# mfkiwl/coxgraph

Hardware: AMD Instinct MI355X
Metric: 640x480 depth frames/sec fused (TSDF, 5 cm voxels) per node; submap registrations/sec reported alongside (higher is better)
Workload: dtype f32; 1 GPU; configs[1]: 1 client per GPU, 640x480 synthetic depth stream, 5 cm voxels, merged integrator semantics (the reference's configured method is fast; bit-exact vs CPU oracle), points resident in HBM; points_per_frame=307200, method=merged, clients=1

## Files before the change

coxgraph_amd/csrc/cox_integrator.hip:

```cpp
#include <hip/hip_runtime.h>

#include <algorithm>
#include <chrono>
#include <cmath>
#include <cstring>
#include <limits>
#include <new>
#include <string>
#include <vector>

#include "../../include/coxgraph_hip_history.h"
#include "../../include/coxgraph_hip_selftest.h"
#include "cox_host.hpp"
#include "cox_plan.hpp"
#include "cox_sort.hpp"
#include "cox_threads.hpp"

using namespace cox;
using cox_plan::IntegratorPlan;
using cox_plan::LayerUpdate;

#include "cox_frame.hpp"
#include "cox_raygen.hpp"
#include "cox_walk.hpp"
#include "cox_pieces.hpp"
#include "cox_fast.hpp"
#include "cox_apply_records.hpp"
#include "cox_apply_tile.hpp"
#include "cox_frontend.hpp"

static_assert(cox_plan::kAxisCapSmall == kAxisCapSmall && cox_plan::kTileShift == kTileShift && cox_plan::kBigChunk == kBigChunk &&
                  cox_plan::kBigChunkMin == kBigChunkMin && cox_plan::kFastMaxRounds == kFastMaxRounds && cox_plan::kFastShortMax == kFastShortMax &&
                  cox_plan::kFastRelaxGroups == kFastRelaxGroups && cox_plan::kCopyGroups == kCopyGroups,
              "cox_plan.hpp decides with the kernels' own constants");

constexpr int kStatRing = 8;
constexpr int kFrameSets = 6;
constexpr int kStageSets = 3;
constexpr int kInputSets = kFrameSets;
using cox_plan::kNumStages;

struct FrameSet {
  FrameParams* d_params = nullptr;
  Counters* cnt = nullptr;
  RayArrays rays{};
  u64* fh_keys = nullptr;
  u32* fh_first = nullptr;
  hipEvent_t done = nullptr;
  hipEvent_t params_copied = nullptr;
  hipEvent_t hand[kNumStages - 1] = {};
  bool used = false;
};
struct BundleSet {
  u32 *pslot = nullptr, *skey[2] = {nullptr, nullptr}, *sval[2] = {nullptr, nullptr}, *bstart = nullptr;
  u32 *hrank = nullptr, *head = nullptr;
  SortInfo* sort_info = nullptr;
  hipEvent_t done = nullptr;
  bool used = false;
};
struct RecordSet {
  u32 *rec_key[2] = {nullptr, nullptr}, *rec_ray[2] = {nullptr, nullptr};
  u32 *piece_front = nullptr, *piece_back = nullptr, *piece_wsum = nullptr;
  uint8_t* lin8 = nullptr;
  u32 *pkey[2] = {nullptr, nullptr}, *pstart[2] = {nullptr, nullptr}, *prl[2] = {nullptr, nullptr};
  u64* pbkey = nullptr;
  u32 *plen = nullptr, *pdest = nullptr;
  u32* touched_slots = nullptr;
// ... 158 lines not shown
  if (I->submitter) {
    I->submitter->wait_outstanding(0);
    const int st = I->submitter->take_status();
    if (st != COX_OK) return st;
  }
  for (int k = 0; k < kNumStages; ++k)
    if (I->st[k] && (k == 0 || I->st[k] != I->st[k - 1])) COX_HIP(hipStreamSynchronize(I->st[k]));
  if (I->st_alt) COX_HIP(hipStreamSynchronize(I->st_alt));
  if (I->st_in) COX_HIP(hipStreamSynchronize(I->st_in));
  if (I->obs) COX_TRY(cox_internal_obs_wait(I->obs));
  return COX_OK;
}

static void drop_graphs(cox_integrator* I) {
  for (auto& row : I->graphs)
    for (hipGraphExec_t& g : row) {
      if (g) (void)hipGraphExecDestroy(g);
      g = nullptr;
    }
}

static int alloc_ray_sets(cox_integrator* I, u32 cap) {
  for (FrameSet& F : I->fs) {
    RayArrays& R = F.rays;
    for (float** p : {&R.px, &R.py, &R.pz, &R.w}) COX_TRY(dev_realloc(I, p, cap));
    for (u32** p : {&R.color, &R.flags, &R.nsteps, &R.rec_off, &R.pbound, &R.piece_off}) COX_TRY(dev_realloc(I, p, cap));
    COX_TRY(dev_realloc(I, &R.key, cap));
    COX_TRY(dev_realloc(I, &R.q, static_cast<size_t>(cap) * 8));
    COX_TRY(dev_realloc(I, &F.fh_keys, static_cast<size_t>(I->fh_cap) + I->fh_cap / 2 + 1));
    F.fh_first = reinterpret_cast<u32*>(F.fh_keys + I->fh_cap);
    COX_HIP(hipMemset(F.fh_keys, 0xFF, sizeof(u64) * I->fh_cap + sizeof(u32) * I->fh_cap));
  }
  for (BundleSet& B : I->bs) {
    for (u32** p : {&B.pslot, &B.skey[0], &B.sval[0], &B.skey[1], &B.sval[1], &B.hrank, &B.bstart}) COX_TRY(dev_realloc(I, p, cap));
    COX_TRY(dev_realloc(I, &B.head, static_cast<size_t>(4) * (cap / kHeadTile + 1)));
  }
  for (int k = 0; k < kInputSets; ++k) {
    COX_TRY(dev_realloc(I, &I->own_xyz[k], static_cast<size_t>(cap) * 3));
    COX_TRY(dev_realloc(I, &I->own_rgba[k], static_cast<size_t>(cap) * 4));
    COX_TRY(dev_realloc(I, &I->own_depth[k], cap));
    COX_TRY(dev_realloc(I, &I->own_depth_rgba[k], static_cast<size_t>(cap) * 4));
  }
  COX_TRY(dev_realloc(I, &I->depth_flag, cap));
  COX_TRY(alloc_sort_ws(I, &I->sort_pts, cap));
  COX_TRY(alloc_sort_ws(I, &I->sort_pts_alt, cap));
  for (ScanWorkspace* ws : {&I->scanws_a, &I->scanws_b, &I->scanws_f}) COX_TRY(dev_realloc(I, &ws->block_sums, scan_num_blocks(cap) + 2));
  return COX_OK;
}
static int alloc_record_sets(cox_integrator* I) {
  const bool pieces = I->plan.walks_pieces(), expand = I->plan.expands_pieces();
  const u32 rcap = I->rcap, piece_cap = I->piece_cap, wave_cap = rcap / 64 + 2;
  for (RecordSet& S : I->rs) {
    if (pieces) {
      COX_TRY(dev_realloc(I, &S.lin8, static_cast<size_t>(piece_cap) * 32));
      for (u32** p : {&S.pkey[0], &S.pstart[0], &S.prl[0], &S.pkey[1], &S.pstart[1], &S.prl[1]}) COX_TRY(dev_realloc(I, p, piece_cap));
    }
    if (expand) {
      COX_TRY(dev_realloc(I, &S.pbkey, piece_cap));
      COX_TRY(dev_realloc(I, &S.plen, piece_cap));
      COX_TRY(dev_realloc(I, &S.pdest, piece_cap));
      S.big_chunk_cap = static_cast<u32>(rcap / kBigChunkMin) + kBigCap + 1u;
      COX_TRY(dev_realloc(I, &S.big_chunks, S.big_chunk_cap));
    }
    if (!pieces || expand) {
      COX_TRY(dev_realloc(I, &S.rec_key[0], rcap));
      COX_TRY(dev_realloc(I, &S.rec_ray[0], rcap));
    }
// ... 142 lines not shown
        return e;
      }
      hipEvent_t e = nullptr;
      return hipEventCreate(&e) == hipSuccess ? e : nullptr;
    };
    e0 = take();
    e1 = take();
    if (!e0 || !e1) {
      e0 = e1 = nullptr;
      return;
    }
    (void)hipEventRecord(e0, s);
  }
  ~TimedRegion() {
    if (!e0) return;
    (void)hipEventRecord(e1, s);
    I->class_events[cls].emplace_back(e0, e1);
  }
};

struct StageCtx {
  cox_integrator* I;
  FrameSet* F;
  BundleSet* B;
  RecordSet* S;
  int slot;
  u64 frame;
  const u32* n_dev = nullptr;
};

static LayerView layer_view(const cox_layer* Lh) {
  return LayerView{Lh->voxels, Lh->ht_keys, Lh->ht_vals, Lh->ht_stamp, Lh->ht_ord, Lh->block_keys, Lh->d_nblocks, Lh->ht_cap - 1, static_cast<u32>(Lh->capacity)};
}
static int points_sort_passes(const cox_integrator* I) { return (ceil_log2(next_pow2(static_cast<u64>(I->pcap) + 1)) + 1 + 10) / 11; }

static int stage_hash(const StageCtx& c, hipStream_t s) {
  cox_integrator* I = c.I;
  FrameSet& F = *c.F;
  BundleSet& B = *c.B;
  const bool by_value = (I->method == COX_METHOD_MERGED) && !I->graphs_on;
  if (!by_value) {
    COX_HIP(hipMemcpyAsync(F.d_params, &I->h_params[c.slot], sizeof(FrameParams), hipMemcpyHostToDevice, s));
    if (c.n_dev) hipLaunchKernelGGL(k_params_count, dim3(1), dim3(1), 0, s, F.d_params, c.n_dev);
  }
  COX_HIP(hipMemsetAsync(F.cnt, 0, sizeof(Counters), s));
  if (I->method == COX_METHOD_MERGED) {
    const u32 n = I->pcap;
    {
      TimedRegion t(I, COX_KC_BUNDLE_HASH, s);
      const bool self_clean = !I->cfg.enable_anti_grazing;
      if (!self_clean) COX_HIP(hipMemsetAsync(F.fh_keys, 0xFF, sizeof(u64) * I->fh_cap + sizeof(u32) * I->fh_cap, s));
      hipLaunchKernelGGL(k_bundle_insert, grid_for(n), dim3(256), 0, s, F.d_params, I->h_params[c.slot], by_value ? 1 : 0, c.n_dev, F.fh_keys, F.fh_first,
                         I->fh_cap - 1, B.pslot, F.cnt);
    }
  }
  return COX_OK;
}
static int stage_point_sort(const StageCtx& c, hipStream_t s) {
  cox_integrator* I = c.I;
  FrameSet& F = *c.F;
  BundleSet& B = *c.B;
  if (I->method == COX_METHOD_MERGED) {
    const u32 n = I->pcap;
    const SortWorkspace& ws = (I->st_alt && (c.slot & 1)) ? I->sort_pts_alt : I->sort_pts;
    const bool counted = static_cast<u64>(n) <= static_cast<u64>(kRsMaxTiles) * kRsTile;
    {
      TimedRegion t(I, COX_KC_BUNDLE_HASH, s);
      hipLaunchKernelGGL(k_bundle_keys, grid_for(n, kHeadTile), dim3(kKeysThreads), 0, s, F.d_params, F.fh_keys, F.fh_first, B.pslot, B.skey[0], B.sval[0], B.hrank, B.head,
                         B.sort_info, counted ? ws.counts : nullptr, ws.totals);
    }
    const bool self_clean = !I->cfg.enable_anti_grazing;
    const BundleBounds bounds{F.d_params, B.head, B.hrank, B.pslot, B.bstart, F.cnt, self_clean ? F.fh_keys : nullptr, F.fh_first, I->fh_cap - 1};
    TimedRegion t(I, COX_KC_POINT_SORT, s);
    (void)radix_sort_pairs<11, BundleBounds>(B.skey[0], B.sval[0], B.skey[1], B.sval[1], &F.d_params->n_points, n, n, 0, true, points_sort_passes(I), ws, B.sort_info,
                                             s, nullptr, nullptr, counted, bounds);
  }
  return COX_OK;
}
static FrameBlocks frame_blocks(const cox_integrator* I, const RecordSet& S) { return FrameBlocks{S.ft_keys, S.ft_ord, S.touched_slots, I->layer->ht_cap - 1}; }
static void record_walk(const StageCtx& c, hipStream_t s) {
  cox_integrator* I = c.I;
  const IntegratorPlan& P = I->plan;
  FrameSet& F = *c.F;
  RecordSet& S = *c.S;
  const u32 fh_mask = I->fh_cap - 1;
  const FrameBlocks FB = frame_blocks(I, S);
  if (P.small_axis_cap)
    hipLaunchKernelGGL(k_touch_wave<kAxisCapSmall>, dim3(P.grid_touch), dim3(256), 0, s, F.d_params, F.rays, FB, S.rec_key[1], I->rcap, F.cnt, F.fh_keys, fh_mask);
  else
    hipLaunchKernelGGL(k_touch_wave<kAxisCapLarge>, dim3(2048), dim3(256), 0, s, F.d_params, F.rays, FB, S.rec_key[1], I->rcap, F.cnt, F.fh_keys, fh_mask);
  hipLaunchKernelGGL(k_emit_wave, dim3(P.grid_touch), dim3(256), 0, s, F.d_params, F.rays, FB, S.rec_key[1], S.rec_key[0], S.rec_ray[0], I->rcap, F.cnt, S.sort_info,
                     F.fh_keys, fh_mask, P.emit_flags());
}
static bool binds_in_apply(const cox_integrator* I) { return I->method == COX_METHOD_MERGED && I->plan.layer_update == LayerUpdate::RecordTiles; }
static void bind_blocks(const StageCtx& c, hipStream_t s) {
  cox_integrator* I = c.I;
  if (binds_in_apply(I)) return;
  hipLaunchKernelGGL(k_bind_blocks, dim3(16), dim3(256), 0, s, layer_view(I->layer), frame_blocks(I, *c.S), c.S->ord_info, c.F->cnt, I->layer->d_err);
}
static int stage_merge(const StageCtx& c, hipStream_t s) {
  cox_integrator* I = c.I;
  FrameSet& F = *c.F;
  BundleSet& B = *c.B;
  const u32 n = I->pcap;
  if (I->method == COX_METHOD_MERGED) {
    BundleView V{{B.skey[0], B.skey[1]}, {B.sval[0], B.sval[1]}, B.sort_info};
    {
      TimedRegion t(I, COX_KC_MERGE, s);
      hipLaunchKernelGGL(k_bundle_merge, dim3(I->plan.grid_merge), dim3(256), 0, s, F.d_params, V, B.bstart, F.rays, F.cnt,
                         I->plan.walks_pieces() ? (I->plan.small_axis_cap ? kAxisCapSmall : kAxisCapLarge) : 0u);
    }
    const bool odd = I->st_alt && (c.slot & 1);
    const ScanWorkspace& ws = odd ? I->scanws_a : I->scanws_b;
    if (!I->plan.walks_pieces()) {
      hipLaunchKernelGGL(k_scan_small, dim3(1), dim3(1024), 0, s, F.rays.nsteps, F.rays.rec_off, &F.cnt->n_ray_slots, I->pcap, &F.cnt->n_records);
    } else if (I->plan.small_axis_cap) {
      hipLaunchKernelGGL(k_scan_small2, dim3(1), dim3(1024), 0, s, F.rays.nsteps, F.rays.rec_off, &F.cnt->n_records, F.rays.pbound, F.rays.piece_off,
                         &F.cnt->n_piece_slots, &F.cnt->n_ray_slots, I->pcap);
    } else {
      exclusive_scan_u32(F.rays.nsteps, F.rays.rec_off, &F.cnt->n_ray_slots, I->pcap, I->pcap, &F.cnt->n_records, ws, s);
      exclusive_scan_u32(F.rays.pbound, F.rays.piece_off, &F.cnt->n_ray_slots, I->pcap, I->pcap, &F.cnt->n_piece_slots, ws, s);
    }
  } else {
    hipLaunchKernelGGL(k_rays_simple, grid_for(n), dim3(256), 0, s, F.d_params, F.rays, F.cnt);
  }
  return COX_OK;
}
static int stage_touch(const StageCtx& c, hipStream_t s) {
  cox_integrator* I = c.I;
  const IntegratorPlan& P = I->plan;
  FrameSet& F = *c.F;
  RecordSet& S = *c.S;
  const LayerView L = layer_view(I->layer);
  const u32 fh_mask = I->fh_cap - 1;
  if (P.walk_on_raygen) {
    bind_blocks(c, s);
    return COX_OK;
  }
  TimedRegion t_walk(I, COX_KC_TOUCH_EMIT, s);
  if (P.walks_pieces()) {
    const PieceArrays PA{S.pkey[0], S.pstart[0], S.prl[0], S.pbkey};
#define COX_LAUNCH_WALK(CAP, DEFER)                                                                                                                       \
  hipLaunchKernelGGL((k_touch_pieces<CAP, DEFER>), dim3(2048), dim3(256), 0, s, F.d_params, F.rays, L, S.touched_slots, S.lin8, PA, I->rcap, I->piece_cap, \
// ... 1179 lines not shown
```

coxgraph_amd/csrc/cox_plan.hpp:

```cpp
#pragma once
#include <algorithm>
#include <cmath>
#include <cstdint>
#include <cstdio>
#include <cstdlib>
#include <cstring>
#include <string>

#include "../../include/coxgraph_hip.h"

namespace cox_plan {

#define COX_PLAN_SWITCHES(X)                                                                                                                   \
  X(APPLY) X(APPLY_WAVE) X(BIG_CHUNK) X(BUCKETS) X(COPY_THREADS) X(DEBUG) X(DEPTH_CONVERT) X(FAST_CAP) X(FAST_FENCE) X(FAST_GROUPS)             \
  X(FAST_ROUNDS) X(FAST_SEQUENTIAL) X(FAST_STREAMS) X(GRAPH) X(GRID_APPLY) X(GRID_APPLY_WAVE) X(GRID_MERGE) X(GRID_TOUCH) X(H2D) X(H2D_GROUPS) \
  X(INPUT_STREAM) X(NO_GRAPH) X(PARTITION) X(QUEUES) X(RECORD_CAP) X(SPLIT_TILES) X(STREAMS) X(STREAM_MAP) X(SUBMIT_THREAD) X(TILE) X(TIMELINE) X(WALK)       \
  X(WAVE_TILE_MAX)
#define COX_PLAN_ENUM(n) k##n,
#define COX_PLAN_NAME(n) "COX_" #n,
enum Switch { COX_PLAN_SWITCHES(COX_PLAN_ENUM) kNumSwitches };
constexpr const char* kSwitchNames[kNumSwitches] = {COX_PLAN_SWITCHES(COX_PLAN_NAME)};
#undef COX_PLAN_ENUM
#undef COX_PLAN_NAME

constexpr uint32_t kAxisCapSmall = 128;
constexpr uint32_t kTileShift = 8, kBigChunk = 4096, kBigChunkMin = 1024;
constexpr int kFastMaxRounds = 8;
constexpr uint32_t kFastCap0Max = 32, kFastShortMax = 32, kFastRelaxGroups = 128;
constexpr int kCopyGroups = 8;
constexpr int kAmpleQueues = 0;
constexpr int kMaxQueueBudget = 64;
constexpr int kNumStages = 6;

enum class LayerUpdate {
  RecordsFullSort,
  RecordTiles,
  PiecesExpand,
  PiecesApply,
};

struct FastPlan {
  int streams = 3;
  int rounds = 2;
  uint32_t cap0 = 8, cap1 = 16;
  uint32_t relax_groups = kFastRelaxGroups;
  int fences = 1;
  bool force_sequential = false;
};

struct IntegratorPlan {
  LayerUpdate layer_update = LayerUpdate::RecordTiles;
  bool bucket_partition = true;
  uint32_t tile_shift = kTileShift;
  bool wave_apply = true;
  bool split_big_tiles = true;
  uint32_t big_chunk = kBigChunk, wave_tile_max = 512;
  uint32_t grid_apply = 8192, grid_apply_wave = 2048, grid_merge = 4096, grid_touch = 2048;
  uint32_t steps_max = 0;
  bool small_axis_cap = false;
  uint32_t record_cap = 0;
  int stage_stream[kNumStages] = {0, 0, 0, 1, 1, 2};
  bool alt_raygen_stream = false;
  bool input_stream = true;
  int n_streams = 0;
  bool walk_on_raygen = false;
  bool use_graphs = false;
  bool submit_thread = true;
  int copy_threads = 3;
  bool h2d_kernel = false;
  int h2d_groups = kCopyGroups;
  bool depth_convert_on_input_stream = false;
  std::string timeline;
  bool debug = false;
  FastPlan fast;

  bool walks_pieces() const { return layer_update == LayerUpdate::PiecesExpand || layer_update == LayerUpdate::PiecesApply; }
  bool tile_apply() const { return layer_update == LayerUpdate::RecordTiles || layer_update == LayerUpdate::PiecesExpand; }
  bool expands_pieces() const { return layer_update == LayerUpdate::PiecesExpand; }
  int n_stage_streams() const { return stage_stream[kNumStages - 1] + 1; }
  int emit_flags() const { return layer_update == LayerUpdate::RecordTiles ? static_cast<int>(tile_shift | (bucket_partition ? 256u : 0u)) : 0; }
  int record_sort_passes() const { return layer_update == LayerUpdate::RecordsFullSort ? 3 : bucket_partition ? 1 : 2; }
};

inline uint32_t max_steps_per_ray(const cox_tsdf_config& cfg, float voxel_size) {
  const double reach = static_cast<double>(cfg.max_ray_length_m) + static_cast<double>(cfg.default_truncation_distance);
  const double per_axis = std::floor(reach / static_cast<double>(voxel_size)) + 3.0;
  return static_cast<uint32_t>(std::min(3.0 * per_axis + 1.0, 1.0e6));
}

template <typename Lookup>
IntegratorPlan resolve_plan(int method, const cox_tsdf_config& cfg, float voxel_size, Lookup env, int hw_queues = kAmpleQueues) {
  const char* v[kNumSwitches];
  for (int k = 0; k < kNumSwitches; ++k) v[k] = env(kSwitchNames[k]);
  auto is = [&](Switch s, const char* word) { return v[s] && std::strcmp(v[s], word) == 0; };
  auto num = [&](Switch s) { return std::atoi(v[s]); };
  const bool merged = method == COX_METHOD_MERGED, fast = method == COX_METHOD_FAST;

  IntegratorPlan p;
  p.steps_max = max_steps_per_ray(cfg, voxel_size);
  p.small_axis_cap = (p.steps_max - 1) / 3 + 2 <= kAxisCapSmall;

  const bool may_walk_pieces = merged && !cfg.enable_anti_grazing;
  p.bucket_partition = v[kBUCKETS] ? num(kBUCKETS) != 0 : p.small_axis_cap;
  if (is(kAPPLY, "records")) {
    p.layer_update = LayerUpdate::RecordsFullSort;
  } else if (may_walk_pieces && is(kAPPLY, "pieces")) {
    p.layer_update = LayerUpdate::PiecesApply;
  } else if (may_walk_pieces) {
    const bool pieces = v[kPARTITION] ? is(kPARTITION, "pieces") : !p.small_axis_cap;
    p.layer_update = pieces ? LayerUpdate::PiecesExpand : LayerUpdate::RecordTiles;
    if (v[kTILE]) p.tile_shift = num(kTILE) == 9 ? 9u : 8u;
  }
  if (v[kRECORD_CAP] && !fast && !p.walks_pieces() && num(kRECORD_CAP) > 0) p.record_cap = static_cast<uint32_t>(num(kRECORD_CAP));
  if (v[kAPPLY_WAVE]) p.wave_apply = num(kAPPLY_WAVE) != 0;
  if (v[kSPLIT_TILES]) p.split_big_tiles = num(kSPLIT_TILES) != 0;
  if (v[kBIG_CHUNK]) p.big_chunk = static_cast<uint32_t>(std::max<int>(kBigChunkMin, num(kBIG_CHUNK)));
  if (v[kWAVE_TILE_MAX]) p.wave_tile_max = num(kWAVE_TILE_MAX) == 256 ? 256u : 512u;
  if (v[kGRID_APPLY]) p.grid_apply = static_cast<uint32_t>(std::max(1, num(kGRID_APPLY)));
  if (v[kGRID_APPLY_WAVE]) p.grid_apply_wave = static_cast<uint32_t>(std::max(8, num(kGRID_APPLY_WAVE)));
  if (v[kGRID_MERGE]) p.grid_merge = static_cast<uint32_t>(std::max(1, num(kGRID_MERGE)));
  if (v[kGRID_TOUCH]) p.grid_touch = static_cast<uint32_t>(std::max(1, num(kGRID_TOUCH)));

  static const int kTwo[kNumStages] = {0, 0, 0, 1, 1, 1};
  static const int kStaged[kNumStages] = {0, 0, 1, 2, 2, 3};
  static const int kSix[kNumStages] = {0, 1, 2, 3, 4, 5};
  static const int kParity[kNumStages] = {0, 0, 0, 1, 1, 2};
  static const int kUpdateHeavy[kNumStages] = {0, 0, 0, 1, 2, 3};
  static const int kFast[kNumStages] = {0, 1, 1, 2, 2, 2};
  static const int kOne[kNumStages] = {0, 0, 0, 0, 0, 0};
  int width = 4;
  if (v[kSTREAMS] && (num(kSTREAMS) == 2 || num(kSTREAMS) == 4 || num(kSTREAMS) == 6)) width = num(kSTREAMS);
  const bool chosen = v[kSTREAM_MAP] || v[kSTREAMS];
  const bool three_p = is(kSTREAMS, "3p");
  const bool update_heavy = !chosen && merged && p.expands_pieces();
// ... 86 lines not shown
```

coxgraph_amd/csrc/cox_raygen.hpp:

```cpp
#pragma once

__global__ void __launch_bounds__(256) k_rays_simple(const FrameParams* __restrict__ Pp, RayArrays R,
                                                     Counters* cnt) {
  const FrameParams P = *Pp;
  const u32 seq = blockIdx.x * blockDim.x + threadIdx.x;
  if (seq == 0) cnt->n_ray_slots = P.n_points;
  if (seq >= P.n_points) return;
  const u32 idx = mixed_index(seq, P.n_points);
  const F3 p{P.xyz[3 * idx], P.xyz[3 * idx + 1], P.xyz[3 * idx + 2]};
  bool clearing = false;
  const bool valid = point_valid(P, p, &clearing);
  u32 nsteps = 0, flags = 0;
  if (valid) {
    const F3 pg = transform_point(P, p);
    Dda d;
    dda_setup(d, P, pg, clearing);
    if (d.range_error) atomicOr(&cnt->err, kErrRange);
    nsteps = d.nsteps;
    flags = 1u | (clearing ? 2u : 0u);
    R.px[seq] = pg.x;
    R.py[seq] = pg.y;
    R.pz[seq] = pg.z;
    R.w[seq] = voxel_weight(P, p);
    R.color[seq] = pack_rgba_wire(P.rgba, idx);
// ... 60 lines not shown
    if (mine) my_leader = leader;
    if (lane == leader) {
      is_leader = true;
      group_min = mn;
    }
    todo &= ~peers;
  }
  u32 sl = kInvalid;
  if (is_leader) {
    bool fresh;
    sl = ht_insert(fh_keys, fh_mask, key, &fresh);
    if (sl == kInvalid)
      atomicOr(&cnt->err, kErrTable);
    else if (__hip_atomic_load(&fh_first[sl], __ATOMIC_RELAXED, __HIP_MEMORY_SCOPE_AGENT) > group_min)
      atomicMin(&fh_first[sl], group_min);
  }
  const u32 got = static_cast<u32>(__shfl(static_cast<int>(sl), static_cast<int>(my_leader), 64));
  const u32 slot = valid ? got : kInvalid;
  if (idx < n_points) pslot[idx] = slot;
  const u64 m = __ballot(valid && slot != kInvalid);
  if (lane == 0 && m) atomicAdd(&cnt->shard[(idx >> 6) & 63u][kShValid], static_cast<u32>(__popcll(m)));
}
__global__ void k_params_count(FrameParams* __restrict__ Pp, const u32* __restrict__ n_dev) {
  const u32 n = min(*n_dev, Pp->n_points);
  Pp->n_points = n;
  Pp->np2 = pow2_above(n);
}
constexpr u32 kHeadTile = kRsTile;
constexpr u32 kHeadTileShift = 11;
static_assert((1u << kHeadTileShift) == kHeadTile, "kHeadTile");
constexpr u32 kKeysThreads = 1024;
constexpr u32 kKeysWaves = kKeysThreads / 64;
constexpr u32 kHeadRounds = kHeadTile / kKeysThreads;
__global__ void __launch_bounds__(kKeysThreads) k_bundle_keys(const FrameParams* __restrict__ Pp, const u64* __restrict__ fh_keys, const u32* __restrict__ fh_first,
                                                     const u32* __restrict__ pslot, u32* __restrict__ skey, u32* __restrict__ sval, u32* __restrict__ hrank,
                                                     u32* __restrict__ tile_heads, SortInfo* sort_info, u32* __restrict__ counts ,
                                                     u32* __restrict__ totals) {
  __shared__ u32 h[1u << 11];
  __shared__ u32 wcnt[kHeadRounds][kKeysWaves];
  const u32 n = Pp->n_points, np2 = Pp->np2;
  u32 nbits = 1;
  while ((1u << (nbits - 1)) < np2) ++nbits;
  if (blockIdx.x == 0 && threadIdx.x == 0) {
    sort_info->nbits = nbits;
    sort_info->parity = 0;
    sort_info->base = 0;
  }
  const u32 tile = blockIdx.x;
  if (tile * kHeadTile >= n) return;
  int shift;
  u32 dbits;
  (void)rs_pass_digits<11>(nbits, 0, &shift, &dbits);
  const u32 kDigits = 1u << dbits;
  if (counts) {
    for (u32 d = threadIdx.x; d < kDigits; d += kKeysThreads) h[d] = 0;
    __syncthreads();
  }
  const u32 lane = lane_id(), wave = threadIdx.x >> 6;
  const u64 lower = (1ull << lane) - 1ull;
  u32 rank_in_wave[kHeadRounds];
  u32 head_mask = 0, clr_mask = 0;
#pragma unroll
  for (u32 q = 0; q < kHeadRounds; ++q) {
    const u32 seq = tile * kHeadTile + q * kKeysThreads + threadIdx.x;
    u32 slot = kInvalid;
    if (seq < n) slot = pslot[mixed_index(seq, n)];
    u32 k = kInvalid;
    bool head = false, clr = false;
    if (slot != kInvalid) {
      const u32 first = fh_first[slot];
      clr = (fh_keys[slot] >> 63) != 0;
      k = first + (clr ? np2 : 0u);
      head = first == seq;
    }
    if (seq < n) {
      skey[seq] = k;
      sval[seq] = seq;
      if (counts) atomicAdd(&h[(k >> shift) & (kDigits - 1)], 1u);
    }
    const u64 b0 = __ballot(head && !clr), b1 = __ballot(head && clr), bv = __ballot(slot != kInvalid);
    rank_in_wave[q] = static_cast<u32>(__popcll((clr ? b1 : b0) & lower));
    head_mask |= (head ? 1u : 0u) << q;
    clr_mask |= (clr ? 1u : 0u) << q;
    if (lane == 0) wcnt[q][wave] = static_cast<u32>(__popcll(b0)) | (static_cast<u32>(__popcll(b1)) << 8) | (static_cast<u32>(__popcll(bv)) << 16);
  }
  __syncthreads();
  u32 run0 = 0, run1 = 0, runv = 0;
#pragma unroll
  for (u32 q = 0; q < kHeadRounds; ++q) {
#pragma unroll
    for (u32 w = 0; w < kKeysWaves; ++w) {
      if (w == wave && ((head_mask >> q) & 1u)) hrank[tile * kHeadTile + q * kKeysThreads + threadIdx.x] = (((clr_mask >> q) & 1u) ? run1 : run0) + rank_in_wave[q];
      const u32 c = wcnt[q][w];
      run0 += c & 255u;
      run1 += (c >> 8) & 255u;
      runv += c >> 16;
    }
  }
  if (threadIdx.x == 0) {
    tile_heads[4 * tile + 0] = run0;
    tile_heads[4 * tile + 1] = run1;
    tile_heads[4 * tile + 2] = runv;
  }
  if (counts) {
    for (u32 d = threadIdx.x; d < kDigits; d += kKeysThreads) {
      const u32 c = h[d];
      counts[static_cast<size_t>(tile) * kDigits + d] = c;
      if (c) atomicAdd(&totals[d], c);
    }
  }
}
struct BundleView {
  const u32* key[2];
  const u32* val[2];
  const SortInfo* info;
};
constexpr u32 kHeadLdsTiles = 2048;
struct BundleBounds {
  static constexpr bool kActive = true;
  static constexpr u32 kLdsWords = 2 * kHeadLdsTiles + 8;
  const FrameParams* Pp;
  const u32* tile_heads;
  const u32* hrank;
  const u32* pslot;
  u32* bstart;
  Counters* cnt;
  u64* fh_keys;
  u32* fh_first;
  u32 fh_mask;
  __device__ __forceinline__ void begin(u32 n, u32* lds) const {
    u32* scratch = lds + 2 * kHeadLdsTiles;
    const u32 n_tiles = (n + kHeadTile - 1) / kHeadTile;
    u32 carry = 0;
    for (u32 cls = 0; cls < 2; ++cls) {
      for (u32 b = 0; b < n_tiles; b += 256) {
        const u32 t = b + threadIdx.x;
        const u32 v = (t < n_tiles) ? tile_heads[4 * t + cls] : 0u;
        u32 tot;
        const u32 ex = block_exclusive_scan<4>(v, &tot, scratch);
        if (t < n_tiles && t < kHeadLdsTiles) lds[cls * kHeadLdsTiles + t] = carry + ex;
        carry += tot;
      }
    }
    if (blockIdx.x == 0) {
      u32 v = 0;
      for (u32 t = threadIdx.x; t < n_tiles; t += 256) v += tile_heads[4 * t + 2];
      u32 n_valid;
      (void)block_exclusive_scan<4>(v, &n_valid, scratch);
      if (threadIdx.x == 0) {
        cnt->n_rays = carry;
        cnt->n_ray_slots = carry;
        cnt->n_sorted_valid = n_valid;
      }
    }
    if (threadIdx.x == 0) {
      scratch[4] = n;
      scratch[5] = Pp->np2;
    }
    __syncthreads();
  }
  struct Fetched {
    u32 ord, slot;
  };
  __device__ __forceinline__ bool wants(u32 key, u32 val, const u32* lds) const {
    const u32 np2 = lds[2 * kHeadLdsTiles + 5];
    return key != kInvalid && (key & (np2 - 1u)) == val;
  }
  __device__ __forceinline__ Fetched fetch(u32 key, u32 val, const u32* lds) const {
    const u32 n = lds[2 * kHeadLdsTiles + 4], np2 = lds[2 * kHeadLdsTiles + 5];
    const u32 cls = key >= np2 ? 1u : 0u;
    const u32 tile = val >> kHeadTileShift;
    u32 ord;
    if (tile < kHeadLdsTiles) {
      ord = lds[cls * kHeadLdsTiles + tile];
    } else {
      ord = lds[cls * kHeadLdsTiles + kHeadLdsTiles - 1];
      for (u32 t = kHeadLdsTiles - 1; t < tile; ++t) ord += tile_heads[4 * t + cls];
    }
    ord += hrank[val];
    return Fetched{ord < n ? ord : kInvalid, fh_keys ? pslot[mixed_index(val, n)] : kInvalid};
  }
  __device__ __forceinline__ void commit(const Fetched& f, u32 pos) const {
    if (f.ord != kInvalid) bstart[f.ord] = pos;
    if (f.slot <= fh_mask) {
      fh_keys[f.slot] = kEmptyKey;
      fh_first[f.slot] = 0xFFFFFFFFu;
    }
  }
};

typedef float MergeOp __attribute__((ext_vector_type(4)));

__device__ __forceinline__ u32 piece_bound(const Dda& d, u32 axis_cap) {
  const u32 ns = d.nsteps;
  if (ns == 0) return 0;
  const u32 gen = ns + 1;
  const u32 g0 = min(d.n_axis[0] + 2, gen), g1 = min(d.n_axis[1] + 2, gen), g2 = min(d.n_axis[2] + 2, gen);
  if (d.sgn[0] == 0 || d.sgn[1] == 0 || d.sgn[2] == 0 || g0 > axis_cap || g1 > axis_cap || g2 > axis_cap || ns > 3 * axis_cap) return ns;
  const u32 b = (ns + 63) / 64 + (d.n_axis[2] + 1) + ((d.n_axis[0] + 1) / 16 + 1) + ((d.n_axis[1] + 1) / 16 + 1) + 4;
  return min(b, ns);
}

__global__ void __launch_bounds__(256) k_bundle_merge(const FrameParams* __restrict__ Pp, BundleView V, const u32* __restrict__ bstart, RayArrays R, Counters* cnt,
                                                      u32 piece_axis_cap) {
  const FrameParams P = *Pp;
  const u32 np2 = P.np2;
  const float* __restrict__ xyz = P.xyz;
  const uint8_t* __restrict__ rgba = P.rgba;
  typedef const float __attribute__((address_space(1))) * GlobalF32;
  typedef const u32 __attribute__((address_space(1))) * GlobalU32;
  const GlobalF32 gxyz = (GlobalF32)xyz;
  const GlobalU32 grgba = (GlobalU32)rgba;
  const u32 spar = uniform_u32(V.info->parity & 1u);
  const u32* __restrict__ skey = V.key[spar];
  const u32* __restrict__ sval = V.val[spar];
  __shared__ MergeOp ops[4][64][4];
  const u32 n_bundles = uniform_u32(cnt->n_rays);
  const u32 n_valid = uniform_u32(cnt->n_sorted_valid);
  const u32 tid = blockIdx.x * blockDim.x + threadIdx.x;
  const u32 nthreads = gridDim.x * blockDim.x;
  const u32 lane = lane_id();
  const u32 role = lane & 3u;
  MergeOp(*tbl)[4] = ops[threadIdx.x >> 6];
  for (u32 task = uniform_u32(tid >> 6); task < 2 * n_bundles; task += nthreads >> 6) {
    const u32 m = task >> 1;
    const bool colour_wave = (task & 1u) != 0;
    const u32 begin = uniform_u32(bstart[m]);
    const u32 next_start = uniform_u32(bstart[min(m + 1u, n_bundles - 1u)]);
    const u32 end = (m + 1 < n_bundles) ? next_start : n_valid;
    if (colour_wave && rgba == nullptr) {
      if (lane == 0) {
        R.color[m] = 0u;
        reinterpret_cast<u32*>(R.q)[static_cast<size_t>(m) * 8u + 5u] = 0u;
      }
      continue;
    }
    auto gather = [&](bool has, u32 sv, float& x, float& y, float& z, u32& c) {
      x = 0.0f;
      y = 0.0f;
      z = 0.0f;
      c = 0u;
      if (has) {
        const u32 idx = mixed_index(sv, P.n_points);
        x = gxyz[3 * idx];
        y = gxyz[3 * idx + 1];
        z = gxyz[3 * idx + 2];
        if (colour_wave) c = grgba[idx];
      }
    };
    const u32 key0 = skey[begin];
    const u32 sv_a = (begin + lane < end) ? sval[begin + lane] : 0u;
    u32 sv_b = (begin + 64u + lane < end) ? sval[begin + 64u + lane] : 0u;
    float npx, npy, npz;
    u32 ncol;
    gather(begin + lane < end, sv_a, npx, npy, npz, ncol);
    const bool clearing = uniform_u32(key0) >= np2;
    if (!colour_wave && lane == 0) atomicMax(&cnt->shard[m & 63u][kShMaxBundle], end - begin);
    float val = 0.0f;
    float W = 0.0f;
    u64 key = 0;
    bool done = false;
    for (u32 base = begin; base < end && !done; base += 64) {
      const u32 i = base + lane;
      const u32 cnt_in = min(64u, end - base);
      const float px = npx, py = npy, pz = npz;
      const u32 col = rgba_wire_order(ncol);
      const float w = (i < end) ? voxel_weight(P, F3{px, py, pz}) : 0.0f;
      gather(i + 64u < end, sv_b, npx, npy, npz, ncol);
      sv_b = (i + 128u < end) ? sval[i + 128u] : 0u;
      if (base == begin && !colour_wave) {
        const F3 pg = transform_point(P, F3{readlane_f32(px, 0), readlane_f32(py, 0), readlane_f32(pz, 0)});
        key = pack_key(grid_index(pg.x * P.voxel_size_inv), grid_index(pg.y * P.voxel_size_inv), grid_index(pg.z * P.voxel_size_inv));
      }
      bool used = (lane < cnt_in) && !(w < kEps);
      if (clearing) {
        const u64 um = __ballot(used);
        used = used && (lane == static_cast<u32>(__ffsll(static_cast<long long>(um))) - 1u);
        if (um) done = true;
      }
      float Wpre;
      const u64 in_mask = (cnt_in == 64) ? ~0ull : ((1ull << cnt_in) - 1ull);
      if (!clearing && (__ballot(w == 1.0f) & in_mask) == in_mask && W == truncf(W) && W < 8388608.0f) {
        Wpre = W + static_cast<float>(lane);
      } else {
        float run = W;
        Wpre = W;
        const u64 used_mask = __ballot(used);
        for (u32 k = 0; k < cnt_in; ++k) {
          if (lane == k) Wpre = run;
          const float wk = readlane_f32(w, k);
          if ((used_mask >> k) & 1ull) run += wk;
        }
      }
      const float den = Wpre + w;
      const float Wnext = used ? den : Wpre;
      const bool d_ok = !used || (den >= 9.094947e-13f && den <= 1.0995116e12f);
      {
        MergeOp* row = tbl[lane];
        const MergeOp ident{1.0f, 0.0f, 1.0f, 1.0f};
        if (!used) {
#pragma unroll
          for (u32 c = 0; c < 4; ++c) row[c] = ident;
        } else if (!colour_wave) {
          const float r0 = __builtin_amdgcn_rcpf(den);
          const float r = __builtin_fmaf(__builtin_fmaf(-den, r0, 1.0f), r0, r0);
          row[0] = MergeOp{Wpre, px * w, den, r};
          row[1] = MergeOp{Wpre, py * w, den, r};
          row[2] = MergeOp{Wpre, pz * w, den, r};
          row[3] = ident;
        } else {
          const float fa = Wpre / den, fb = w / den;
#pragma unroll
          for (u32 c = 0; c < 4; ++c) row[c] = MergeOp{fa, static_cast<float>(static_cast<int>((col >> (8u * c)) & 255u)) * fb, 1.0f, 0.0f};
        }
      }
      wave_lds_handover();
      MergeOp nxt = tbl[0][role];
      if (!colour_wave) {
        const float val_in = val;
        float n_lo = 1.0f, n_hi = 1.0f;
        MergeOp a0 = tbl[0][role], a1 = tbl[1][role], a2 = tbl[2][role], a3 = tbl[3][role];
#define COX_MERGE_STEP(op)                                  \
  {                                                         \
    const float N = val * (op).x + (op).y;                  \
    n_lo = fminf(n_lo, fabsf(N));                           \
    n_hi = fmaxf(n_hi, fabsf(N));                           \
    const float q0 = N * (op).w;                            \
    const float e0 = __builtin_fmaf(-(op).z, q0, N);        \
    const float q1 = __builtin_fmaf(e0, (op).w, q0);        \
    const float e1 = __builtin_fmaf(-(op).z, q1, N);        \
    val = __builtin_fmaf(e1, (op).w, q1);                   \
// ... 32 lines not shown
        }
      } else {
#define COX_COLOUR_STEP(op)                                 \
  {                                                         \
    const float x = val * (op).x + (op).y;                  \
    const float t = truncf(x);                              \
    val = (x - t >= 0.5f) ? t + 1.0f : t;                   \
  }
        MergeOp a0 = tbl[0][role], a1 = tbl[1][role], a2 = tbl[2][role], a3 = tbl[3][role];
        for (u32 k = 0; k < cnt_in; k += 8) {
          const u32 kb = (k + 4) & 63u;
          const MergeOp b0 = tbl[kb][role], b1 = tbl[kb + 1][role], b2 = tbl[kb + 2][role], b3 = tbl[kb + 3][role];
          __builtin_amdgcn_sched_barrier(0);
          COX_COLOUR_STEP(a0)
          COX_COLOUR_STEP(a1)
          COX_COLOUR_STEP(a2)
          COX_COLOUR_STEP(a3)
          __builtin_amdgcn_sched_barrier(0);
          const u32 ka = (k + 8) & 63u;
          a0 = tbl[ka][role];
          a1 = tbl[ka + 1][role];
          a2 = tbl[ka + 2][role];
          a3 = tbl[ka + 3][role];
          __builtin_amdgcn_sched_barrier(0);
          COX_COLOUR_STEP(b0)
          COX_COLOUR_STEP(b1)
          COX_COLOUR_STEP(b2)
          COX_COLOUR_STEP(b3)
          __builtin_amdgcn_sched_barrier(0);
        }
#undef COX_COLOUR_STEP
      }
      wave_lds_handover();
      W = readlane_f32(Wnext, cnt_in - 1);
    }
    if (colour_wave) {
      u32 mcolor = 0;
#pragma unroll
      for (u32 c = 0; c < 4; ++c) mcolor |= (static_cast<u32>(static_cast<int>(readlane_f32(val, c))) & 255u) << (8u * c);
      if (lane == 0) {
        R.color[m] = mcolor;
        reinterpret_cast<u32*>(R.q)[static_cast<size_t>(m) * 8u + 5u] = mcolor;
      }
    } else {
      const float mx = readlane_f32(val, 0), my = readlane_f32(val, 1), mz = readlane_f32(val, 2);
      if (lane == 0) {
        const F3 pg = transform_point(P, F3{mx, my, mz});
        Dda d;
        dda_setup(d, P, pg, clearing);
        if (d.range_error) atomicOr(&cnt->err, kErrRange);
        R.px[m] = pg.x;
        R.py[m] = pg.y;
        R.pz[m] = pg.z;
        R.w[m] = W;
        R.flags[m] = 1u | (clearing ? 2u : 0u);
        R.key[m] = key;
        R.nsteps[m] = d.nsteps;
        if (piece_axis_cap) R.pbound[m] = piece_bound(d, piece_axis_cap);
        {
          const F3 dv = pg - F3{P.tx, P.ty, P.tz};
          typedef float F4 __attribute__((ext_vector_type(4)));
          F4* q = reinterpret_cast<F4*>(R.q + static_cast<size_t>(m) * 8u);
          q[0] = F4{dv.x, dv.y, dv.z, sqrtf(dot3(dv, dv))};
          R.q[static_cast<size_t>(m) * 8u + 4u] = W;
        }
      }
    }
// ... 3 lines not shown
```

Measured before the change: 8343 frames/s.

## Replace multi-pass bundle point sort with single 12-bit bucket pass

After: 8141 frames/s. -2.4%, worse.

```diff
diff --git a/coxgraph_amd/csrc/cox_integrator.hip b/coxgraph_amd/csrc/cox_integrator.hip
--- a/coxgraph_amd/csrc/cox_integrator.hip
+++ b/coxgraph_amd/csrc/cox_integrator.hip
@@ -33,6 +33,7 @@
                   cox_plan::kBigChunkMin == kBigChunkMin && cox_plan::kFastMaxRounds == kFastMaxRounds && cox_plan::kFastShortMax == kFastShortMax &&
                   cox_plan::kFastRelaxGroups == kFastRelaxGroups && cox_plan::kCopyGroups == kCopyGroups,
               "cox_plan.hpp decides with the kernels' own constants");
+static_assert(cox_plan::kBundleBitsMin == 6 && cox_plan::kBundleBitsMax == kRsMaxDigitBits, "the bundle bucket pass is one pass of the 12-bit digit kernels");
 
 constexpr int kStatRing = 8;
 constexpr int kFrameSets = 6;
@@ -257,7 +258,8 @@
     COX_HIP(hipMemset(F.fh_keys, 0xFF, sizeof(u64) * I->fh_cap + sizeof(u32) * I->fh_cap));
   }
   for (BundleSet& B : I->bs) {
-    for (u32** p : {&B.pslot, &B.skey[0], &B.sval[0], &B.skey[1], &B.sval[1], &B.hrank, &B.bstart}) COX_TRY(dev_realloc(I, p, cap));
+    for (u32** p : {&B.pslot, &B.skey[0], &B.sval[0], &B.skey[1], &B.sval[1], &B.hrank}) COX_TRY(dev_realloc(I, p, cap));
+    COX_TRY(dev_realloc(I, &B.bstart, static_cast<size_t>(cap) * 2));
     COX_TRY(dev_realloc(I, &B.head, static_cast<size_t>(4) * (cap / kHeadTile + 1)));
   }
   for (int k = 0; k < kInputSets; ++k) {
@@ -466,6 +468,7 @@
 static LayerView layer_view(const cox_layer* Lh) {
   return LayerView{Lh->voxels, Lh->ht_keys, Lh->ht_vals, Lh->ht_stamp, Lh->ht_ord, Lh->block_keys, Lh->d_nblocks, Lh->ht_cap - 1, static_cast<u32>(Lh->capacity)};
 }
+static bool bundle_buckets(const cox_integrator* I) { return I->plan.bundle_buckets && I->fh_cap < (1u << 30); }
 static int points_sort_passes(const cox_integrator* I) { return (ceil_log2(next_pow2(static_cast<u64>(I->pcap) + 1)) + 1 + 10) / 11; }
 
 static int stage_hash(const StageCtx& c, hipStream_t s) {
@@ -498,16 +501,28 @@
     const u32 n = I->pcap;
     const SortWorkspace& ws = (I->st_alt && (c.slot & 1)) ? I->sort_pts_alt : I->sort_pts;
     const bool counted = static_cast<u64>(n) <= static_cast<u64>(kRsMaxTiles) * kRsTile;
+    const bool buckets = bundle_buckets(I);
+    const u32 bits = I->plan.bundle_bits;
     {
       TimedRegion t(I, COX_KC_BUNDLE_HASH, s);
-      hipLaunchKernelGGL(k_bundle_keys, grid_for(n, kHeadTile), dim3(kKeysThreads), 0, s, F.d_params, F.fh_keys, F.fh_first, B.pslot, B.skey[0], B.sval[0], B.hrank, B.head,
-                         B.sort_info, counted ? ws.counts : nullptr, ws.totals);
+      if (buckets)
+        hipLaunchKernelGGL(k_bundle_keys<true>, grid_for(n, kHeadTile), dim3(kKeysThreads), 0, s, F.d_params, F.fh_keys, F.fh_first, B.pslot, B.skey[0], B.sval[0], B.hrank,
+                           B.head, B.sort_info, counted ? ws.counts : nullptr, ws.totals, bits);
+      else
+        hipLaunchKernelGGL(k_bundle_keys<false>, grid_for(n, kHeadTile), dim3(kKeysThreads), 0, s, F.d_params, F.fh_keys, F.fh_first, B.pslot, B.skey[0], B.sval[0], B.hrank,
+                           B.head, B.sort_info, counted ? ws.counts : nullptr, ws.totals, 0u);
     }
     const bool self_clean = !I->cfg.enable_anti_grazing;
-    const BundleBounds bounds{F.d_params, B.head, B.hrank, B.pslot, B.bstart, F.cnt, self_clean ? F.fh_keys : nullptr, F.fh_first, I->fh_cap - 1};
     TimedRegion t(I, COX_KC_POINT_SORT, s);
-    (void)radix_sort_pairs<11, BundleBounds>(B.skey[0], B.sval[0], B.skey[1], B.sval[1], &F.d_params->n_points, n, n, 0, true, points_sort_passes(I), ws, B.sort_info,
-                                             s, nullptr, nullptr, counted, bounds);
+    if (buckets) {
+      const BucketBounds bounds{F.d_params, B.head, B.hrank, B.pslot, B.bstart, F.cnt, self_clean ? F.fh_keys : nullptr, F.fh_first, I->fh_cap - 1, ws.counts, bits};
+      (void)radix_sort_pairs<12, BucketBounds>(B.skey[0], B.sval[0], B.skey[1], B.sval[1], &F.d_params->n_points, n, n, static_cast<int>(bits), false, 1, ws, B.sort_info,
+                                               s, nullptr, nullptr, counted, bounds);
+    } else {
+      const BundleBounds bounds{F.d_params, B.head, B.hrank, B.pslot, B.bstart, F.cnt, self_clean ? F.fh_keys : nullptr, F.fh_first, I->fh_cap - 1};
+      (void)radix_sort_pairs<11, BundleBounds>(B.skey[0], B.sval[0], B.skey[1], B.sval[1], &F.d_params->n_points, n, n, 0, true, points_sort_passes(I), ws, B.sort_info,
+                                               s, nullptr, nullptr, counted, bounds);
+    }
   }
   return COX_OK;
 }
@@ -541,8 +556,11 @@
     BundleView V{{B.skey[0], B.skey[1]}, {B.sval[0], B.sval[1]}, B.sort_info};
     {
       TimedRegion t(I, COX_KC_MERGE, s);
-      hipLaunchKernelGGL(k_bundle_merge, dim3(I->plan.grid_merge), dim3(256), 0, s, F.d_params, V, B.bstart, F.rays, F.cnt,
-                         I->plan.walks_pieces() ? (I->plan.small_axis_cap ? kAxisCapSmall : kAxisCapLarge) : 0u);
+      const u32 piece_axis_cap = I->plan.walks_pieces() ? (I->plan.small_axis_cap ? kAxisCapSmall : kAxisCapLarge) : 0u;
+      if (bundle_buckets(I))
+        hipLaunchKernelGGL(k_bundle_merge<true>, dim3(I->plan.grid_merge), dim3(256), 0, s, F.d_params, V, B.bstart, F.rays, F.cnt, piece_axis_cap);
+      else
+        hipLaunchKernelGGL(k_bundle_merge<false>, dim3(I->plan.grid_merge), dim3(256), 0, s, F.d_params, V, B.bstart, F.rays, F.cnt, piece_axis_cap);
     }
     const bool odd = I->st_alt && (c.slot & 1);
     const ScanWorkspace& ws = odd ? I->scanws_a : I->scanws_b;
diff --git a/coxgraph_amd/csrc/cox_plan.hpp b/coxgraph_amd/csrc/cox_plan.hpp
--- a/coxgraph_amd/csrc/cox_plan.hpp
+++ b/coxgraph_amd/csrc/cox_plan.hpp
@@ -12,7 +12,7 @@
 namespace cox_plan {
 
 #define COX_PLAN_SWITCHES(X)                                                                                                                   \
-  X(APPLY) X(APPLY_WAVE) X(BIG_CHUNK) X(BUCKETS) X(COPY_THREADS) X(DEBUG) X(DEPTH_CONVERT) X(FAST_CAP) X(FAST_FENCE) X(FAST_GROUPS)             \
+  X(APPLY) X(APPLY_WAVE) X(BIG_CHUNK) X(BUCKETS) X(BUNDLE_BITS) X(BUNDLE_SORT) X(COPY_THREADS) X(DEBUG) X(DEPTH_CONVERT) X(FAST_CAP) X(FAST_FENCE) X(FAST_GROUPS)             \
   X(FAST_ROUNDS) X(FAST_SEQUENTIAL) X(FAST_STREAMS) X(GRAPH) X(GRID_APPLY) X(GRID_APPLY_WAVE) X(GRID_MERGE) X(GRID_TOUCH) X(H2D) X(H2D_GROUPS) \
   X(INPUT_STREAM) X(NO_GRAPH) X(PARTITION) X(QUEUES) X(RECORD_CAP) X(SPLIT_TILES) X(STREAMS) X(STREAM_MAP) X(SUBMIT_THREAD) X(TILE) X(TIMELINE) X(WALK)       \
   X(WAVE_TILE_MAX)
@@ -30,6 +30,7 @@
 constexpr int kCopyGroups = 8;
 constexpr int kAmpleQueues = 0;
 constexpr int kMaxQueueBudget = 64;
+constexpr uint32_t kBundleBitsMin = 6, kBundleBitsMax = 12;
 constexpr int kNumStages = 6;
 
 enum class LayerUpdate {
@@ -49,6 +50,8 @@
 };
 
 struct IntegratorPlan {
+  bool bundle_buckets = false;
+  uint32_t bundle_bits = kBundleBitsMax;
   LayerUpdate layer_update = LayerUpdate::RecordTiles;
   bool bucket_partition = true;
   uint32_t tile_shift = kTileShift;
@@ -100,6 +103,9 @@
   p.steps_max = max_steps_per_ray(cfg, voxel_size);
   p.small_axis_cap = (p.steps_max - 1) / 3 + 2 <= kAxisCapSmall;
 
+  p.bundle_buckets = merged && (is(kBUNDLE_SORT, "buckets") ? true : is(kBUNDLE_SORT, "full") ? false : p.small_axis_cap);
+  if (v[kBUNDLE_BITS]) p.bundle_bits = static_cast<uint32_t>(std::min<int>(kBundleBitsMax, std::max<int>(kBundleBitsMin, num(kBUNDLE_BITS))));
+
   const bool may_walk_pieces = merged && !cfg.enable_anti_grazing;
   p.bucket_partition = v[kBUCKETS] ? num(kBUCKETS) != 0 : p.small_axis_cap;
   if (is(kAPPLY, "records")) {
diff --git a/coxgraph_amd/csrc/cox_raygen.hpp b/coxgraph_amd/csrc/cox_raygen.hpp
--- a/coxgraph_amd/csrc/cox_raygen.hpp
+++ b/coxgraph_amd/csrc/cox_raygen.hpp
@@ -116,25 +116,31 @@
 constexpr u32 kKeysThreads = 1024;
 constexpr u32 kKeysWaves = kKeysThreads / 64;
 constexpr u32 kHeadRounds = kHeadTile / kKeysThreads;
+constexpr u32 kKeyHead = 1u << 30, kKeyClear = 1u << 31, kKeySlotMask = kKeyHead - 1u;
+template <bool kBuckets>
 __global__ void __launch_bounds__(kKeysThreads) k_bundle_keys(const FrameParams* __restrict__ Pp, const u64* __restrict__ fh_keys, const u32* __restrict__ fh_first,
                                                      const u32* __restrict__ pslot, u32* __restrict__ skey, u32* __restrict__ sval, u32* __restrict__ hrank,
                                                      u32* __restrict__ tile_heads, SortInfo* sort_info, u32* __restrict__ counts ,
-                                                     u32* __restrict__ totals) {
-  __shared__ u32 h[1u << 11];
+                                                     u32* __restrict__ totals, u32 bucket_bits) {
+  __shared__ u32 h[1u << (kBuckets ? 12 : 11)];
   __shared__ u32 wcnt[kHeadRounds][kKeysWaves];
   const u32 n = Pp->n_points, np2 = Pp->np2;
   u32 nbits = 1;
-  while ((1u << (nbits - 1)) < np2) ++nbits;
+  if constexpr (kBuckets) {
+    nbits = bucket_bits;
+  } else {
+    while ((1u << (nbits - 1)) < np2) ++nbits;
+  }
   if (blockIdx.x == 0 && threadIdx.x == 0) {
     sort_info->nbits = nbits;
-    sort_info->parity = 0;
+    sort_info->parity = kBuckets ? 1u : 0u;
     sort_info->base = 0;
   }
   const u32 tile = blockIdx.x;
   if (tile * kHeadTile >= n) return;
   int shift;
   u32 dbits;
-  (void)rs_pass_digits<11>(nbits, 0, &shift, &dbits);
+  (void)rs_pass_digits<kBuckets ? 12 : 11>(nbits, 0, &shift, &dbits);
   const u32 kDigits = 1u << dbits;
   if (counts) {
     for (u32 d = threadIdx.x; d < kDigits; d += kKeysThreads) h[d] = 0;
@@ -154,8 +160,8 @@
     if (slot != kInvalid) {
       const u32 first = fh_first[slot];
       clr = (fh_keys[slot] >> 63) != 0;
-      k = first + (clr ? np2 : 0u);
       head = first == seq;
+      k = kBuckets ? (slot | (head ? kKeyHead : 0u) | (clr ? kKeyClear : 0u)) : first + (clr ? np2 : 0u);
     }
     if (seq < n) {
       skey[seq] = k;
@@ -200,7 +206,8 @@
   const SortInfo* info;
 };
 constexpr u32 kHeadLdsTiles = 2048;
-struct BundleBounds {
+template <bool kBuckets>
+struct BundleBoundsT {
   static constexpr bool kActive = true;
   static constexpr u32 kLdsWords = 2 * kHeadLdsTiles + 8;
   const FrameParams* Pp;
@@ -212,6 +219,8 @@
   u64* fh_keys;
   u32* fh_first;
   u32 fh_mask;
+  const u32* offsets = nullptr;
+  u32 bucket_bits = 0;
   __device__ __forceinline__ void begin(u32 n, u32* lds) const {
     u32* scratch = lds + 2 * kHeadLdsTiles;
     const u32 n_tiles = (n + kHeadTile - 1) / kHeadTile;
@@ -244,15 +253,16 @@
     __syncthreads();
   }
   struct Fetched {
-    u32 ord, slot;
+    u32 ord, slot, end;
   };
   __device__ __forceinline__ bool wants(u32 key, u32 val, const u32* lds) const {
+    if constexpr (kBuckets) return key != kInvalid && (key & kKeyHead) != 0;
     const u32 np2 = lds[2 * kHeadLdsTiles + 5];
     return key != kInvalid && (key & (np2 - 1u)) == val;
   }
   __device__ __forceinline__ Fetched fetch(u32 key, u32 val, const u32* lds) const {
     const u32 n = lds[2 * kHeadLdsTiles + 4], np2 = lds[2 * kHeadLdsTiles + 5];
-    const u32 cls = key >= np2 ? 1u : 0u;
+    const u32 cls = kBuckets ? key >> 31 : (key >= np2 ? 1u : 0u);
     const u32 tile = val >> kHeadTileShift;
     u32 ord;
     if (tile < kHeadLdsTiles) {
@@ -262,16 +272,27 @@
       for (u32 t = kHeadLdsTiles - 1; t < tile; ++t) ord += tile_heads[4 * t + cls];
     }
     ord += hrank[val];
-    return Fetched{ord < n ? ord : kInvalid, fh_keys ? pslot[mixed_index(val, n)] : kInvalid};
+    if constexpr (kBuckets) {
+      const u32 next_digit = (key & ((1u << bucket_bits) - 1u)) + 1u;
+      const u32 end = (next_digit >> bucket_bits) ? n : offsets[next_digit];
+      return Fetched{ord < n ? ord : kInvalid, fh_keys ? (key & kKeySlotMask) : kInvalid, end};
+    }
+    return Fetched{ord < n ? ord : kInvalid, fh_keys ? pslot[mixed_index(val, n)] : kInvalid, 0u};
   }
   __device__ __forceinline__ void commit(const Fetched& f, u32 pos) const {
-    if (f.ord != kInvalid) bstart[f.ord] = pos;
+    if constexpr (kBuckets) {
+      if (f.ord != kInvalid) reinterpret_cast<uint2*>(bstart)[f.ord] = make_uint2(pos, f.end);
+    } else {
+      if (f.ord != kInvalid) bstart[f.ord] = pos;
+    }
     if (f.slot <= fh_mask) {
       fh_keys[f.slot] = kEmptyKey;
       fh_first[f.slot] = 0xFFFFFFFFu;
     }
   }
 };
+using BundleBounds = BundleBoundsT<false>;
+using BucketBounds = BundleBoundsT<true>;
 
 typedef float MergeOp __attribute__((ext_vector_type(4)));
 
@@ -285,6 +306,7 @@
   return min(b, ns);
 }
 
+template <bool kBuckets>
 __global__ void __launch_bounds__(256) k_bundle_merge(const FrameParams* __restrict__ Pp, BundleView V, const u32* __restrict__ bstart, RayArrays R, Counters* cnt,
                                                       u32 piece_axis_cap) {
   const FrameParams P = *Pp;
@@ -309,9 +331,16 @@
   for (u32 task = uniform_u32(tid >> 6); task < 2 * n_bundles; task += nthreads >> 6) {
     const u32 m = task >> 1;
     const bool colour_wave = (task & 1u) != 0;
-    const u32 begin = uniform_u32(bstart[m]);
-    const u32 next_start = uniform_u32(bstart[min(m + 1u, n_bundles - 1u)]);
-    const u32 end = (m + 1 < n_bundles) ? next_start : n_valid;
+    u32 begin, end;
+    if constexpr (kBuckets) {
+      const uint2 be = reinterpret_cast<const uint2*>(bstart)[m];
+      begin = uniform_u32(be.x);
+      end = uniform_u32(be.y);
+    } else {
+      begin = uniform_u32(bstart[m]);
+      const u32 next_start = uniform_u32(bstart[min(m + 1u, n_bundles - 1u)]);
+      end = (m + 1 < n_bundles) ? next_start : n_valid;
+    }
     if (colour_wave && rgba == nullptr) {
       if (lane == 0) {
         R.color[m] = 0u;
@@ -332,45 +361,74 @@
         if (colour_wave) c = grgba[idx];
       }
     };
-    const u32 key0 = skey[begin];
+    u32 sk_a = kInvalid, sk_b = kInvalid;
+    if constexpr (kBuckets) {
+      if (begin + lane < end) sk_a = skey[begin + lane];
+      if (begin + 64u + lane < end) sk_b = skey[begin + 64u + lane];
+    }
     const u32 sv_a = (begin + lane < end) ? sval[begin + lane] : 0u;
     u32 sv_b = (begin + 64u + lane < end) ? sval[begin + 64u + lane] : 0u;
+    const u32 key0 = kBuckets ? uniform_u32(sk_a) : skey[begin];
+    const u32 own_key = key0 & ~kKeyHead;
     float npx, npy, npz;
     u32 ncol;
-    gather(begin + lane < end, sv_a, npx, npy, npz, ncol);
-    const bool clearing = uniform_u32(key0) >= np2;
-    if (!colour_wave && lane == 0) atomicMax(&cnt->shard[m & 63u][kShMaxBundle], end - begin);
+    bool nmine = kBuckets ? (sk_a & ~kKeyHead) == own_key : begin + lane < end;
+    gather(nmine, sv_a, npx, npy, npz, ncol);
+    const bool clearing = kBuckets ? (uniform_u32(key0) >> 31) != 0 : uniform_u32(key0) >= np2;
+    if constexpr (!kBuckets)
+      if (!colour_wave && lane == 0) atomicMax(&cnt->shard[m & 63u][kShMaxBundle], end - begin);
+    u32 own_total = 0;
     float val = 0.0f;
     float W = 0.0f;
     u64 key = 0;
     bool done = false;
-    for (u32 base = begin; base < end && !done; base += 64) {
+    u32 base = begin;
+    for (; base < end && !done; base += 64) {
       const u32 i = base + lane;
-      const u32 cnt_in = min(64u, end - base);
+      const bool mine = nmine;
       const float px = npx, py = npy, pz = npz;
       const u32 col = rgba_wire_order(ncol);
-      const float w = (i < end) ? voxel_weight(P, F3{px, py, pz}) : 0.0f;
-      gather(i + 64u < end, sv_b, npx, npy, npz, ncol);
+      const float w = mine ? voxel_weight(P, F3{px, py, pz}) : 0.0f;
+      nmine = kBuckets ? (sk_b & ~kKeyHead) == own_key : i + 64u < end;
+      gather(nmine, sv_b, npx, npy, npz, ncol);
       sv_b = (i + 128u < end) ? sval[i + 128u] : 0u;
+      if constexpr (kBuckets) sk_b = (i + 128u < end) ? skey[i + 128u] : kInvalid;
+      u64 in_mask;
+      u32 cnt_in, span, rank, row_of;
+      if constexpr (kBuckets) {
+        in_mask = __ballot(mine);
+        if (in_mask == 0ull) continue;
+        cnt_in = static_cast<u32>(__popcll(in_mask));
+        span = 64u - static_cast<u32>(__clzll(static_cast<long long>(in_mask)));
+        const u64 lower = (1ull << lane) - 1ull;
+        rank = static_cast<u32>(__popcll(in_mask & lower));
+        row_of = mine ? rank : cnt_in + static_cast<u32>(__popcll(~in_mask & lower));
+        own_total += cnt_in;
+      } else {
+        cnt_in = min(64u, end - base);
+        in_mask = (cnt_in == 64) ? ~0ull : ((1ull << cnt_in) - 1ull);
+        span = cnt_in;
+        rank = lane;
+        row_of = lane;
+      }
       if (base == begin && !colour_wave) {
         const F3 pg = transform_point(P, F3{readlane_f32(px, 0), readlane_f32(py, 0), readlane_f32(pz, 0)});
         key = pack_key(grid_index(pg.x * P.voxel_size_inv), grid_index(pg.y * P.voxel_size_inv), grid_index(pg.z * P.voxel_size_inv));
       }
-      bool used = (lane < cnt_in) && !(w < kEps);
+      bool used = mine && !(w < kEps);
       if (clearing) {
         const u64 um = __ballot(used);
         used = used && (lane == static_cast<u32>(__ffsll(static_cast<long long>(um))) - 1u);
         if (um) done = true;
       }
       float Wpre;
-      const u64 in_mask = (cnt_in == 64) ? ~0ull : ((1ull << cnt_in) - 1ull);
       if (!clearing && (__ballot(w == 1.0f) & in_mask) == in_mask && W == truncf(W) && W < 8388608.0f) {
-        Wpre = W + static_cast<float>(lane);
+        Wpre = W + static_cast<float>(rank);
       } else {
         float run = W;
         Wpre = W;
         const u64 used_mask = __ballot(used);
-        for (u32 k = 0; k < cnt_in; ++k) {
+        for (u32 k = 0; k < span; ++k) {
           if (lane == k) Wpre = run;
           const float wk = readlane_f32(w, k);
           if ((used_mask >> k) & 1ull) run += wk;
@@ -380,7 +438,7 @@
       const float Wnext = used ? den : Wpre;
       const bool d_ok = !used || (den >= 9.094947e-13f && den <= 1.0995116e12f);
       {
-        MergeOp* row = tbl[lane];
+        MergeOp* row = tbl[row_of];
         const MergeOp ident{1.0f, 0.0f, 1.0f, 1.0f};
         if (!used) {
 #pragma unroll
@@ -479,7 +537,17 @@
 #undef COX_COLOUR_STEP
       }
       wave_lds_handover();
-      W = readlane_f32(Wnext, cnt_in - 1);
+      W = readlane_f32(Wnext, span - 1);
+    }
+    if constexpr (kBuckets) {
+      if (!colour_wave) {
+        for (; base < end; base += 64) {
+          const u32 i = base + lane;
+          const u32 k = (i < end) ? skey[i] : kInvalid;
+          own_total += static_cast<u32>(__popcll(__ballot((k & ~kKeyHead) == own_key)));
+        }
+        if (lane == 0) atomicMax(&cnt->shard[m & 63u][kShMaxBundle], own_total);
+      }
     }
     if (colour_wave) {
       u32 mcolor = 0;
```
